# Jittor/JDet

Measured on AMD Instinct MI355X. Metric: img/s S2ANet-R50-FPN train step, 1024x1024 synthetic tiles, higher is better.
Workload: dtype f32; 1 GPU; s2anet_train; model=S2ANet-R50-FPN (configs/s2anet/s2anet_r50_fpn_1x_dota.py), global_batch=2, tile=1024x1024, gts_per_image=64, optimizer=SGD mom 0.9 wd 1e-4 clip 35 + StepLR warm-up (the config's lr), parallelism=dp1 (DDP, RCCL all-reduce)

## Files before the change

### jdet_amd/_lib.py

```python
import ctypes
import os
import subprocess

import torch

_HERE = os.path.dirname(os.path.abspath(__file__))
CSRC = os.path.join(_HERE, "csrc")
LIB_PATH = os.path.join(CSRC, "libjdet_hip.so")

_i, _f, _p, _sz, _l = ctypes.c_int, ctypes.c_float, ctypes.c_void_p, ctypes.c_size_t, ctypes.c_long



class BnParams(ctypes.Structure):
    _fields_ = [("weight", _p), ("bias", _p), ("mean", _p), ("var", _p), ("eps", _f)]


class ConvEpilogue(ctypes.Structure):
    _fields_ = [("mode", _i), ("affine", _i), ("relu", _i), ("bn", BnParams), ("residual", _p), ("grad_out", _p),
                ("act", _p), ("sums", _p)]


class BnSumsJob(ctypes.Structure):
    _fields_ = [("partial", _p), ("rows", _l), ("C", _i), ("gamma", _p), ("grad_gamma", _p), ("grad_beta", _p)]
# ... 98 lines not shown
    "jdet_rip_forward": (_i, [_p, _l, _i, _i, _p, _p]),
    "jdet_rip_backward": (_i, [_p, _p, _p, _l, _i, _i, _p, _p]),
    "jdet_delta2bbox_rotated": (_i, [_p, _p, _i, _i, _p, _p, _f, _p, _p]),
    "jdet_bbox2delta_rotated": (_i, [_p, _p, _i, _p, _p, _p, _p]),
    "jdet_midpoint_offset_decode": (_i, [_p, _p, _l, _p, _p, _f, _p, _p]),
    "jdet_midpoint_offset_encode": (_i, [_p, _p, _l, _p, _p, _p, _p]),
    "jdet_oriented_delta_decode": (_i, [_p, _p, _l, _i, _p, _p, _f, _p, _p]),
    "jdet_oriented_delta_encode": (_i, [_p, _p, _l, _p, _p, _p, _p]),
    "jdet_gliding_targets": (_i, [_p, _p, _l, _p, _p, _p, _p, _p, _p]),
    "jdet_gliding_decode": (_i, [_p, _p, _p, _p, _l, _i, _p, _p, _f, _f, _f, _f, _p, _p, _p]),
    "jdet_gv_delta_encode": (_i, [_p, _p, _l, _p, _p, _p, _p]),
    "jdet_gv_delta_decode": (_i, [_p, _p, _l, _i, _p, _p, _f, _f, _f, _p, _p]),
    "jdet_anchor_targets_rotated": (_i, [_p, _p, _p, _p, _i, _i, _p, _p, _f, _p, _p, _p, _p, _p, _p]),
    "jdet_anchor_targets_rotated_boxes": (_i, [_p, _p, _p, _i, _i, _f, _p, _p, _p, _p, _p, _p]),
    "jdet_obb2hbb2obb": (_i, [_p, _i, _i, _p, _p]),
    "jdet_assign_max_iou_workspace": (_sz, [_i]),
    "jdet_assign_max_iou": (_i, [_p, _i, _i, _f, _f, _f, _f, _i, _i, _p, _i, _p, _p, _p, _p, _sz, _p]),
}

ATSS_SIGNATURES = {
    "jdet_atss_assign_workspace": (_sz, [_i, _i, _i, _i]),
    "jdet_atss_assign": (_i, [_p, _i, _i, _p, _i, _p, _i, _p, _p, _i, _i, _p, _p, _p, _p, _sz, _p]),
}

ROWS_SIGNATURES = {
    "jdet_rows_nonzero_workspace": (_sz, [_i, _i, _i]),
    "jdet_rows_nonzero": (_i, [_p, _i, _i, _i, _i, _p, _p, _p, _p, _p, _sz, _p]),
    "jdet_conv3x3_rows_supported": (_i, [_i, _i]),
    "jdet_conv3x3_wgrad_rows_workers": (_i, [_i, _i]),
    "jdet_conv3x3_wgrad_rows": (_i, [_p, _p, _p, _p, _i, _i, _i, _i, _i, _p, _p]),
    "jdet_conv3x3_dgrad_rows": (_i, [_p, _p, _p, _p, _i, _i, _i, _i, _i, _i, _p, _p]),
}

FCOS_SIGNATURES = {
    "jdet_fcos_targets": (_i, [_p, _p, _i, _p, _p, _p, _i, _i, _i, _i, _i, _f, _p, _p, _p, _p, _p]),
    "jdet_poly_iou_loss": (_i, [_p, _p, _p, _l, _i, _f, _p, _p, _p]),
}

_lib = None

REFERENCE_SORT = 0


def build(force=False, verbose=False):
    cmd = ["make", "-C", CSRC, "-j8"] + (["-B"] if force else [])
    r = subprocess.run(cmd, capture_output=True, text=True)
    if r.returncode != 0:
        raise RuntimeError("building libjdet_hip.so failed:\n" + r.stdout[-4000:] + r.stderr[-4000:])
    if verbose:
        print(r.stdout[-2000:])
    return LIB_PATH


def lib():
    global _lib
    if _lib is None:
        if not os.path.exists(LIB_PATH):
            raise RuntimeError(
                "jdet_amd: %s not found.  Build it with `python -c 'import __graft_entry__ as g; g.build()'` "
                "or `make -C jdet_amd/csrc` (needs hipcc).  There is no CPU fallback." % LIB_PATH)
        l = ctypes.CDLL(LIB_PATH)
        for name, (res, args) in list(SIGNATURES.items()) + list(ATSS_SIGNATURES.items()) + list(ROWS_SIGNATURES.items()) + \
                list(FCOS_SIGNATURES.items()):
            fn = getattr(l, name)
            fn.restype = res
            fn.argtypes = args
        _lib = l
    return _lib


class JDetHipError(RuntimeError):
    pass


_ERR = {-1: "bad argument", -2: "unsupported shape", -3: "workspace too small"}


def check(status, what):
    if status != 0:
        msg = _ERR.get(status, "hipError_t %d" % status)
        raise JDetHipError("%s failed: %s" % (what, msg))


def stream_ptr(t=None):
    if t is not None and t.is_cuda and t.device.index != torch.cuda.current_device():
        torch.cuda.set_device(t.device)
    return torch.cuda.current_stream(t.device if t is not None else None).cuda_stream


def need_device(*tensors):
    for t in tensors:
        if t is None:
            continue
        if not t.is_cuda:
            raise JDetHipError(
                "jdet_amd ops run only on a HIP device (got a %s tensor); there is no CPU fallback "
# ... 53 lines not shown
```

### jdet_amd/csrc/conv_rows.hip

```cpp
#include "conv_mfma.h"
#include "jdet_hip_rows.h"

namespace {

constexpr int kBlk = 256;
constexpr int kFlagRows = 64;

typedef unsigned v4u __attribute__((ext_vector_type(4)));

__global__ __launch_bounds__(256) void rows_flag_kernel(const float* __restrict__ g, long P, int C4,
                                                        uint8_t* __restrict__ flags) {
  const int lane = threadIdx.x & 63, wave = threadIdx.x >> 6;
  const long base = (long)blockIdx.x * kFlagRows + wave * (kFlagRows / 4);
  const v4u* g4 = reinterpret_cast<const v4u*>(g);
  for (int r = 0; r < kFlagRows / 4; r += 4) {
    unsigned acc[4] = {0u, 0u, 0u, 0u};
#pragma unroll
    for (int u = 0; u < 4; u++) {
      const long row = base + r + u;
      if (row < P)
        for (int c = lane; c < C4; c += 64) {
          const v4u v = g4[row * C4 + c];
          acc[u] |= (v[0] | v[1] | v[2] | v[3]) & 0x7fffffffu;
        }
    }
#pragma unroll
    for (int u = 0; u < 4; u++) {
      const long row = base + r + u;
      const bool any = __ballot(acc[u] != 0u) != 0ull;
      if (lane == 0 && row < P) flags[row] = any ? 1 : 0;
    }
  }
}

// ... 226 lines not shown
#pragma unroll
    for (int i = 0; i < TM; i++)
#pragma unroll
      for (int j = 0; j < TN; j++) {
        const unsigned ci = (unsigned)(n0 + wn * 32 * TN + j * 32 + (lane & 31));
        const unsigned co = (unsigned)(m0 + wm * 32 * TM + i * 32 + 4 * (lane >> 5));
        const unsigned base = ((co * 9u + (unsigned)tap) * (unsigned)a.Cin + ci) * 4u;
#pragma unroll
        for (int e = 0; e < 16; e++)
          __builtin_amdgcn_raw_ptr_buffer_atomic_fadd_f32(acc[i][j][e], rgw, (int)base, (int)(cd_row(e) * row_bytes), 0);
      }
    return;
  }
#pragma unroll
  for (int i = 0; i < TM; i++)
#pragma unroll
    for (int j = 0; j < TN; j++) {
      const int ci = n0 + wn * 32 * TN + j * 32 + (lane & 31);
#pragma unroll
      for (int e = 0; e < 16; e++) {
        const int co = m0 + wm * 32 * TM + i * 32 + cd_row(e) + 4 * (lane >> 5);
        if (co < a.Cout && ci < a.Cin) unsafeAtomicAdd(a.gw + ((size_t)co * 9 + tap) * a.Cin + ci, acc[i][j][e]);
      }
    }
}

struct DgradRowsArgs {
  const float* g;
  const float* wd;
  const int* rows;
  const int* count;
  float* gx;
  int N, H, W, Cin, Cout;
};

template <int BK, int KG>
__global__ __launch_bounds__(256 * KG) __attribute__((amdgpu_waves_per_eu(4)))
void conv3x3_dgrad_rows_kernel(DgradRowsArgs a) {
  constexpr int BT = 64;
  constexpr int DEPTH = KG >= 1 ? 1 : 2;
  using TL = MfmaTile<BT, BK, KG>;
  constexpr int T = TL::T, CH = TL::CH, RPP = TL::RPP, PASSES = TL::PASSES, TILE = TL::TILE, QN = TL::QN;
  static_assert(T == 1, "64 x 64 tile");
  __shared__ __attribute__((aligned(16))) char s_raw[4 * TILE];
  const int tid = threadIdx.x, lane = tid & 63, wave = tid >> 6;
  const int P = a.N * a.H * a.W;
  const int KC = a.Cout, NO = a.Cin;
  int cnt = a.count[0];
  cnt = cnt < 0 ? 0 : (cnt > P ? P : cnt);
  const int NT = (NO + BT - 1) / BT;
  const int mtile = (int)((unsigned)blockIdx.x / (unsigned)NT);
  const int m0 = mtile * BT;
  if (m0 >= cnt) return;
  const int n0 = (blockIdx.x - mtile * NT) * BT;
  const __amdgpu_buffer_rsrc_t rx =
      __builtin_amdgcn_make_buffer_rsrc((void*)a.g, 0, (unsigned)((long)P * KC * 4), 0x00020000);
  const __amdgpu_buffer_rsrc_t rw =
      __builtin_amdgcn_make_buffer_rsrc((void*)a.wd, 0, (unsigned)((long)NO * 9 * KC * 4), 0x00020000);
  const int lchunk = tid % CH, lrow = tid / CH;
  int img[PASSES], py[PASSES], px[PASSES];
  bool m_ok[PASSES];
  unsigned wv[PASSES];
  int st_off[PASSES];
  const unsigned hw = (unsigned)(a.H * a.W);
#pragma unroll
  for (int p = 0; p < PASSES; p++) {
    const int row = p * RPP + lrow;
    const int li = m0 + row;
    const unsigned pos = li < cnt ? (unsigned)a.rows[li] : 0xFFFFFFFFu;
// ... 50 lines not shown
    fb_off[qq] = TILE + swz_bytes<BK>(wn * (BT / 2) + frow, chunk);
  }
  v16f acc[T][T];
#pragma unroll
  for (int e = 0; e < 16; e++) acc[0][0][e] = 0.f;

  int tap = 0, c = 0;
  set_tap(0);
  auto advance = [&]() {
    c += BK;
    if (c == KC) {
      c = 0;
      tap++;
      set_tap(tap);
    }
  };
  auto mfma_step = [&](int buf) { ::mfma_step<BT, BK, KG>(s_raw, buf, fa_off, fb_off, acc); };
#include "conv_mfma_loop.inc"
  if (KG == 2) {
    float* red = reinterpret_cast<float*>(s_raw);
    if (kg == 1) {
#pragma unroll
      for (int e = 0; e < 16; e++) red[red_index<T>(wave, lane, 0, 0, e)] = acc[0][0][e];
    }
    __syncthreads();
    if (kg == 1) return;
  }

  const __amdgpu_buffer_rsrc_t ry =
      __builtin_amdgcn_make_buffer_rsrc((void*)a.gx, 0, (unsigned)((long)P * NO * 4), 0x00020000);
  const int lrow0 = m0 + wm * (BT / 2) + 4 * (lane >> 5);
  const int n = n0 + wn * (BT / 2) + (lane & 31);
  unsigned dst[16];
#pragma unroll
  for (int e = 0; e < 16; e++) {
    const int li = lrow0 + cd_row(e);
    const unsigned pos = li < cnt ? (unsigned)a.rows[li] : 0xFFFFFFFFu;
    dst[e] = (pos < (unsigned)P && n < NO) ? (pos * (unsigned)NO + (unsigned)n) * 4u : kOob;
  }
#pragma unroll
  for (int e = 0; e < 16; e++) {
    float v = acc[0][0][e];
    if (KG == 2) v += reinterpret_cast<const float*>(s_raw)[red_index<T>(wave, lane, 0, 0, e)];
    __builtin_amdgcn_raw_buffer_store_b32(__builtin_bit_cast(unsigned, v), ry, dst[e], 0u, 0);
  }
}

inline size_t align16(size_t v) { return (v + 15) & ~(size_t)15; }

inline int wgrad_rows_workers(int Cin, int Cout) {
  const int tm = Cout > 64 ? 2 : 1;
  const long tiles = (long)((Cout + 64 * tm - 1) / (64 * tm)) * ((Cin + 63) / 64) * 9;
  long kw = 1152 / tiles;
  return (int)(kw < 8 ? 8 : (kw > 64 ? 64 : kw));
}

}

JDET_API size_t jdet_rows_nonzero_workspace(int N, int H, int W) {
  if (N <= 0 || H <= 0 || W <= 0) return 0;
  const long P = (long)N * H * W;
  const long nb = (P + kBlk - 1) / kBlk;
  return align16((size_t)P) + sizeof(int32_t) * 2 * (size_t)nb;
}

JDET_API int jdet_rows_nonzero(const float* g_nhwc, int N, int H, int W, int C, uint8_t* flags, int32_t* rows,
                               int32_t* rows_dilated, int32_t* counts, void* workspace, size_t workspace_bytes,
                               jdet_stream_t stream) {
  if (N <= 0 || H <= 0 || W <= 0 || C <= 0) return JDET_E_BADARG;
  if (C % 4 != 0) return JDET_E_UNSUPPORTED;
  const long P = (long)N * H * W;
  if (P * C >= (1L << 30)) return JDET_E_UNSUPPORTED;
  if (!g_nhwc || !flags || !rows || !rows_dilated || !counts) return JDET_E_BADARG;
  if (((uintptr_t)g_nhwc & 15) || (((uintptr_t)rows | (uintptr_t)rows_dilated | (uintptr_t)counts) & 3))
    return JDET_E_BADARG;
  if (!workspace || workspace_bytes < jdet_rows_nonzero_workspace(N, H, W)) return JDET_E_WORKSPACE;
// ... 23 lines not shown
                                     const int32_t* count, int N, int H, int W, int Cin, int Cout, float* gw_krsc,
                                     jdet_stream_t stream) {
  if (N <= 0 || H <= 0 || W <= 0 || Cin <= 0 || Cout <= 0) return JDET_E_BADARG;
  if (!jdet_conv3x3_rows_supported(Cin, Cout)) return JDET_E_UNSUPPORTED;
  const long P = (long)N * H * W;
  if ((P + BKW) * (Cin > Cout ? Cin : Cout) >= (1L << 30)) return JDET_E_UNSUPPORTED;
  if (!x_nhwc || !gy_nhwc || !rows || !count || !gw_krsc) return JDET_E_BADARG;
  if ((((uintptr_t)x_nhwc) | ((uintptr_t)gy_nhwc)) & 15 || (((uintptr_t)rows | (uintptr_t)count) & 3)) return JDET_E_BADARG;
  const int tm = Cout > 64 ? 2 : 1;
  const int kw = wgrad_rows_workers(Cin, Cout);
  const unsigned grid = (unsigned)(((Cout + 64 * tm - 1) / (64 * tm)) * ((Cin + 63) / 64) * 9 * kw);
  WgradRowsArgs a{x_nhwc, gy_nhwc, rows, count, gw_krsc, N, H, W, Cin, Cout, kw};
  hipStream_t st = (hipStream_t)stream;
  if (tm == 2) hipLaunchKernelGGL((conv3x3_wgrad_rows_kernel<2>), dim3(grid), dim3(256), 0, st, a);
  else hipLaunchKernelGGL((conv3x3_wgrad_rows_kernel<1>), dim3(grid), dim3(256), 0, st, a);
  return jdet_launch_status();
}

JDET_API int jdet_conv3x3_dgrad_rows(const float* gy_nhwc, const float* wd_crsk, const int32_t* rows,
                                     const int32_t* count, int N, int H, int W, int Cin, int Cout, int zero_first,
                                     float* gx_nhwc, jdet_stream_t stream) {
  if (N <= 0 || H <= 0 || W <= 0 || Cin <= 0 || Cout <= 0) return JDET_E_BADARG;
  if (!jdet_conv3x3_rows_supported(Cin, Cout)) return JDET_E_UNSUPPORTED;
  const long P = (long)N * H * W;
  if (P * (Cin > Cout ? Cin : Cout) >= (1L << 30)) return JDET_E_UNSUPPORTED;
  if (!gy_nhwc || !wd_crsk || !rows || !count || !gx_nhwc) return JDET_E_BADARG;
  if ((((uintptr_t)gy_nhwc) | ((uintptr_t)wd_crsk)) & 15 || (((uintptr_t)rows | (uintptr_t)count | (uintptr_t)gx_nhwc) & 3))
    return JDET_E_BADARG;
  hipStream_t st = (hipStream_t)stream;
  if (zero_first) {
    const int e = jdet_zero_async(gx_nhwc, sizeof(float) * (size_t)P * Cin, st);
    if (e) return e;
  }
  DgradRowsArgs a{gy_nhwc, wd_crsk, rows, count, gx_nhwc, N, H, W, Cin, Cout};
  const unsigned grid = (unsigned)(((P + 63) / 64) * ((Cin + 63) / 64));
  if (Cout % 32 == 0) hipLaunchKernelGGL((conv3x3_dgrad_rows_kernel<32, 2>), dim3(grid), dim3(512), 0, st, a);
  else hipLaunchKernelGGL((conv3x3_dgrad_rows_kernel<16, 1>), dim3(grid), dim3(256), 0, st, a);
  return jdet_launch_status();
}
```

### jdet_amd/models/roi_heads/s2anet_head.py

```python
import os

import torch
from torch import nn
try:
    from torch.nn.utils.stateless import _reparametrize_module
except ImportError:
    _reparametrize_module = None

from jdet_amd.models.boxes.anchor_generator import AnchorGeneratorRotatedS2ANet
from jdet_amd.models.boxes.anchor_target import anchor_target, images_to_levels
from jdet_amd.models.boxes.box_ops import delta2bbox_rotated
from jdet_amd.models.utils.level_pack import LevelPack

HEAD_STREAMS = os.environ.get("JDET_HEAD_STREAMS", "0") == "1"
FUSED_PACK_MASK = os.environ.get("JDET_PACK_FUSED_MASK", "1") == "1"
_SIDE = {}


def _side_stream(device):
    s = _SIDE.get(device)
    if s is None:
        s = _SIDE[device] = torch.cuda.Stream(device)
    return s
from jdet_amd.models.utils.modules import ConvModule
# ... 109 lines not shown
        normal_init(self.fam_reg, std=0.01)
        normal_init(self.fam_cls, std=0.01, bias=bias_cls)
        self.align_conv.init_weights()
        normal_init(self.or_conv, std=0.01)
        for m in self.odm_reg_convs:
            normal_init(m.conv, std=0.01)
        for m in self.odm_cls_convs:
            normal_init(m.conv, std=0.01)
        normal_init(self.odm_cls, std=0.01, bias=bias_cls)
        normal_init(self.odm_reg, std=0.01)

    def _towers(self, x, convs, mask=None, rows=None):
        for conv in convs:
            y = conv.masked(x, rows) if rows is not None and hasattr(conv, "masked") else None
            if y is not None:
                x = y
                continue
            x = conv(x)
            if mask is not None:
                x = x * mask
        return x

    def _fam(self, x, mask=None, rows=None):
        fam_bbox_pred = conv_module(self.fam_reg, self._towers(x, self.fam_reg_convs, mask, rows))
        fam_cls_score = conv_module(self.fam_cls, self._towers(x, self.fam_cls_convs, mask, rows)) if self.training else None
        return fam_cls_score, fam_bbox_pred

    def _refine(self, x, fam_bbox_pred, stride):
        num_level = self.anchor_strides.index(stride)
        init_anchors = self._init_anchors(num_level, tuple(fam_bbox_pred.shape[-2:]), x.device)
        refine_anchor = bbox_decode(fam_bbox_pred.detach(), init_anchors, self.target_means, self.target_stds)
        return refine_anchor, self.align_conv(x, refine_anchor, stride)

    def _odm(self, align_feat, mask=None, rows=None):
        or_feat = self.or_conv(align_feat)
        if mask is not None:
            or_feat = or_feat * mask
        odm_cls_feat = self.or_pool(or_feat) if self.with_orconv else or_feat
        odm_cls_score = conv_module(self.odm_cls, self._towers(odm_cls_feat, self.odm_cls_convs, mask, rows))
        odm_bbox_pred = conv_module(self.odm_reg, self._towers(or_feat, self.odm_reg_convs, mask, rows))
        return odm_cls_score, odm_bbox_pred

    def forward_single(self, x, stride):
        fam_cls_score, fam_bbox_pred = self._fam(x)
        refine_anchor, align_feat = self._refine(x, fam_bbox_pred, stride)
        odm_cls_score, odm_bbox_pred = self._odm(align_feat)
        return fam_cls_score, fam_bbox_pred, refine_anchor, odm_cls_score, odm_bbox_pred

    def forward_packed(self, xs, strides):
        pack = LevelPack.cached([tuple(x.shape[-2:]) for x in xs], xs[0].device)
        mask = pack.mask.to(xs[0].dtype)
        rows = pack.row_mask(xs[0].shape[0]) if FUSED_PACK_MASK and xs[0].dtype == torch.float32 else None
        fam_cls_p, fam_box_p = self._fam(pack.pack(xs), mask, rows)
        fam_box = pack.unpack(fam_box_p)
        fam_cls = pack.unpack(fam_cls_p) if fam_cls_p is not None else [None] * len(xs)
        refined = [self._refine(x, b, stride) for x, b, stride in zip(xs, fam_box, strides)]
        odm_cls_p, odm_box_p = self._odm(pack.pack([r[1] for r in refined]), mask, rows)
        odm_cls, odm_box = pack.unpack(odm_cls_p), pack.unpack(odm_box_p)
        return [(fam_cls[i], fam_box[i], refined[i][0], odm_cls[i], odm_box[i]) for i in range(len(xs))]

    def get_refine_anchors(self, featmap_sizes, refine_anchors, img_metas, is_train=True, device=None):
        num_levels = len(featmap_sizes)
        refine_anchors_list = []
        for img_id in range(len(img_metas)):
            refine_anchors_list.append([refine_anchors[i][img_id].reshape(-1, 5) for i in range(num_levels)])
        valid_flag_list = self._valid_flags(featmap_sizes, img_metas, device) if is_train else []
        return refine_anchors_list, valid_flag_list

    def loss(self, fam_cls_scores, fam_bbox_preds, refine_anchors, odm_cls_scores, odm_bbox_preds, gt_bboxes,
             gt_labels, img_metas, gt_bboxes_ignore=None):
        cfg = self.train_cfg.copy()
        featmap_sizes = [tuple(featmap.shape[-2:]) for featmap in odm_cls_scores]
        assert len(featmap_sizes) == len(self.anchor_generators)
        device = odm_cls_scores[0].device
        anchor_list, valid_flag_list = self.get_init_anchors(featmap_sizes, img_metas, device)
        num_level_anchors = [anchors.size(0) for anchors in anchor_list[0]]
        need_anchors = cfg.fam_cfg.get("reg_decoded_bbox", False) or cfg.odm_cfg.get("reg_decoded_bbox", False)
        all_anchor_list = [None] * len(num_level_anchors)
        if need_anchors:
            concat_anchor_list = [torch.cat(anchor_list[i]) for i in range(len(anchor_list))]
            all_anchor_list = images_to_levels(concat_anchor_list, num_level_anchors)

        label_channels = self.cls_out_channels if self.use_sigmoid_cls else 1
        cls_reg_targets = anchor_target(anchor_list, valid_flag_list, gt_bboxes, img_metas, self.target_means,
                                        self.target_stds, cfg.fam_cfg, gt_bboxes_ignore_list=gt_bboxes_ignore,
                                        gt_labels_list=gt_labels, label_channels=label_channels,
                                        sampling=self.sampling)
        if cls_reg_targets is None:
            return None
        labels_list, label_weights_list, bbox_targets_list, bbox_weights_list, num_total_pos, num_total_neg = \
            cls_reg_targets
        num_total_samples = num_total_pos + num_total_neg if self.sampling else num_total_pos
        losses_fam_cls, losses_fam_bbox = multi_apply(
            self.loss_fam_single, fam_cls_scores, fam_bbox_preds, all_anchor_list, labels_list, label_weights_list,
            bbox_targets_list, bbox_weights_list, num_total_samples=num_total_samples, cfg=cfg.fam_cfg)

        refine_anchors_list, valid_flag_list = self.get_refine_anchors(featmap_sizes, refine_anchors, img_metas,
                                                                       device=device)
        num_level_anchors = [anchors.size(0) for anchors in refine_anchors_list[0]]
        all_anchor_list = [None] * len(num_level_anchors)
        if need_anchors:
            concat_anchor_list = [torch.cat(refine_anchors_list[i]) for i in range(len(refine_anchors_list))]
            all_anchor_list = images_to_levels(concat_anchor_list, num_level_anchors)
        cls_reg_targets = anchor_target(refine_anchors_list, valid_flag_list, gt_bboxes, img_metas, self.target_means,
                                        self.target_stds, cfg.odm_cfg, gt_bboxes_ignore_list=gt_bboxes_ignore,
                                        gt_labels_list=gt_labels, label_channels=label_channels,
                                        sampling=self.sampling)
        if cls_reg_targets is None:
            return None
        (labels_list, label_weights_list, bbox_targets_list, bbox_weights_list, num_total_pos, num_total_neg) = \
            cls_reg_targets
        num_total_samples = num_total_pos + num_total_neg if self.sampling else num_total_pos
        losses_odm_cls, losses_odm_bbox = multi_apply(
            self.loss_odm_single, odm_cls_scores, odm_bbox_preds, all_anchor_list, labels_list, label_weights_list,
            bbox_targets_list, bbox_weights_list, num_total_samples=num_total_samples, cfg=cfg.odm_cfg)
        return dict(loss_fam_cls=losses_fam_cls, loss_fam_bbox=losses_fam_bbox, loss_odm_cls=losses_odm_cls,
                    loss_odm_bbox=losses_odm_bbox)

    def loss_fam_single(self, fam_cls_score, fam_bbox_pred, anchors, labels, label_weights, bbox_targets,
                        bbox_weights, num_total_samples, cfg):
        return self._loss_single(self.loss_fam_cls, self.loss_fam_bbox, fam_cls_score, fam_bbox_pred, anchors, labels,
                                 label_weights, bbox_targets, bbox_weights, num_total_samples, cfg)

    def loss_odm_single(self, odm_cls_score, odm_bbox_pred, anchors, labels, label_weights, bbox_targets,
                        bbox_weights, num_total_samples, cfg):
        return self._loss_single(self.loss_odm_cls, self.loss_odm_bbox, odm_cls_score, odm_bbox_pred, anchors, labels,
                                 label_weights, bbox_targets, bbox_weights, num_total_samples, cfg)

    def get_bboxes(self, fam_cls_scores, fam_bbox_preds, refine_anchors, odm_cls_scores, odm_bbox_preds, img_metas,
                   rescale=True):
        assert len(odm_cls_scores) == len(odm_bbox_preds)
        cfg = self.test_cfg.copy()
        featmap_sizes = [tuple(featmap.shape[-2:]) for featmap in odm_cls_scores]
        num_levels = len(odm_cls_scores)
        refine_anchors = self.get_refine_anchors(featmap_sizes, refine_anchors, img_metas, is_train=False)
        result_list = []
        for img_id in range(len(img_metas)):
            cls_score_list = [odm_cls_scores[i][img_id].detach() for i in range(num_levels)]
            bbox_pred_list = [odm_bbox_preds[i][img_id].detach() for i in range(num_levels)]
            img_shape = img_metas[img_id]["img_shape"]
# ... 3 lines not shown
        return result_list

    def _level_outputs(self, feats):
        small = [i for i, f in enumerate(feats)
                 if f.is_cuda and f.shape[-2] * f.shape[-1] <= self.pack_max_positions]
        outs = [None] * len(feats)
        side = None
        if len(small) >= 2:
            if (HEAD_STREAMS and _reparametrize_module is not None and len(small) < len(feats)
                    and torch.is_grad_enabled() and not torch.cuda.is_current_stream_capturing()):
                side = _side_stream(feats[0].device)
                main = torch.cuda.current_stream(feats[0].device)
                side.wait_stream(main)
            if side is not None:
                alias = {n: p.view_as(p) for n, p in self.named_parameters() if p.requires_grad}
                with torch.cuda.stream(side), _reparametrize_module(self, alias):
                    packed = self.forward_packed([feats[i] for i in small], [self.anchor_strides[i] for i in small])
            else:
                packed = self.forward_packed([feats[i] for i in small], [self.anchor_strides[i] for i in small])
            for i, o in zip(small, packed):
                outs[i] = o
        for i, f in enumerate(feats):
            if outs[i] is None:
                outs[i] = self.forward_single(f, self.anchor_strides[i])
        if side is not None:
            main.wait_stream(side)
            for i in small:
                feats[i].record_stream(side)
                for t in outs[i]:
                    if torch.is_tensor(t):
                        t.record_stream(main)
        return tuple(map(list, zip(*outs)))

    def forward(self, feats, targets):
        outs = self._level_outputs(feats)
        if self.training:
            return self.loss(*outs, *self.parse_targets(targets))
        return self.get_bboxes(*outs, self.parse_targets(targets, is_train=False))

    execute = forward


def bbox_decode(bbox_preds, anchors, means=[0, 0, 0, 0, 0], stds=[1, 1, 1, 1, 1]):
    num_imgs, _, H, W = bbox_preds.shape
    deltas = bbox_preds.permute(0, 2, 3, 1).reshape(num_imgs * H * W, 5)
    rois = anchors.unsqueeze(0).expand(num_imgs, H * W, 5).reshape(num_imgs * H * W, 5)
    bboxes = delta2bbox_rotated(rois, deltas, means, stds, wh_ratio_clip=1e-6)
    return bboxes.reshape(num_imgs, H, W, 5)


class AlignConv(nn.Module):
    def __init__(self, in_channels, out_channels, kernel_size=3, deformable_groups=1):
        super().__init__()
        self.kernel_size = kernel_size
        self.deform_conv = DeformConv(in_channels, out_channels, kernel_size=kernel_size,
                                      padding=(kernel_size - 1) // 2, deformable_groups=deformable_groups)
        self.relu = nn.ReLU()

    def init_weights(self):
        normal_init(self.deform_conv, std=0.01)

    @torch.no_grad()
    def get_offset(self, anchors, featmap_size, stride):
        dtype, device = anchors.dtype, anchors.device
        feat_h, feat_w = featmap_size
        if anchors.is_cuda and dtype == torch.float32:
            from jdet_amd import _lib as L
# ... 37 lines not shown
```

### jdet_amd/ops/conv_igemm.py

```python
import os
import weakref

import torch

from jdet_amd import _lib as L


def supported(cin, cout):
    return bool(L.lib().jdet_conv3x3_igemm_supported(int(cin), int(cout)))


def weight_krsc(weight):
    return L.f32c(weight.permute(0, 2, 3, 1))


def conv3x3_nhwc(x_nhwc, w_krsc, bias=None, relu=False, rowmask=None, offset=None, tile=0):
    L.need_device(x_nhwc, w_krsc, bias, rowmask, offset)
    N, H, W, Cin = x_nhwc.shape
    Cout = w_krsc.shape[0]
    if w_krsc.shape[1:] != (3, 3, Cin):
        raise ValueError("weight %r does not match input channels %d" % (tuple(w_krsc.shape), Cin))
    if offset is not None and tuple(offset.shape) != (N, 18, H, W):
        raise ValueError("offset must be (N, 18, H, W), got %r" % (tuple(offset.shape),))
    x_nhwc, w_krsc = L.f32c(x_nhwc), L.f32c(w_krsc)
# ... 238 lines not shown
        out = torch.empty((N, H, W, Cin), dtype=torch.float32, device=gy_nhwc.device)
    L.check(L.lib().jdet_conv3x3_dgrad_rows(L.ptr(gy_nhwc), L.ptr(wd_crsk), L.ptr(rows), count_ptr, N, H, W, Cin, Cout,
                                            int(zero), L.ptr(out), L.stream_ptr(gy_nhwc)), "jdet_conv3x3_dgrad_rows")
    return out


def _rows_dgrad_weight(weight):
    if torch.cuda.is_current_stream_capturing() or not weight.is_cuda:
        return weight.detach().flip(2, 3).permute(1, 2, 3, 0).contiguous()
    wd = dgrad_weight(weight)
    st = _DGRAD_BANKS.get(weight.device)
    if st is None or st["bank"] is None or id(weight) not in st["items"]:
        return dgrad_weight_fresh(weight)
    tid = torch._C._current_graph_task_id()
    if tid < 0 or st.get("pass") != tid:
        st["bank"].refresh()
        st["pass"] = tid
    return wd


def dgrad_weight_fresh(weight):
    return weight.detach().flip(2, 3).permute(1, 2, 3, 0).contiguous()


def _rows_backward(g, x, weight, need_x, need_w):
    gn, xn = L.f32c(g.permute(0, 2, 3, 1)), L.f32c(x.permute(0, 2, 3, 1))
    _, rows, drows, counts = rows_nonzero(gn)
    gx = gw = None
    if need_w:
        gw = shared_wgrad(weight, xn, gn, rows=(rows, counts.data_ptr()))
    if need_x:
        gx = conv3x3_dgrad_rows_nhwc(gn, _rows_dgrad_weight(weight), drows, counts.data_ptr() + 4).permute(0, 3, 1, 2)
    return gx, gw


CONV1X1_GEMM = os.environ.get("JDET_CONV1X1_GEMM", "1") == "1"


def _is_1x1(x, weight, stride, padding, groups):
    return (CONV1X1_GEMM and tuple(weight.shape[2:]) == (1, 1) and tuple(stride) == (1, 1) and tuple(padding) == (0, 0)
            and groups == 1 and x.is_cuda and x.dtype == torch.float32 and weight.shape[0] >= 64
            and x.is_contiguous(memory_format=torch.channels_last))


class _ConvBiasAct(torch.autograd.Function):

    @staticmethod
    def forward(ctx, x, weight, bias, relu, stride, padding, dilation, groups, igemm, rowmask=None, row_sparse=False):
        k1 = _is_1x1(x, weight, stride, padding, groups)
        if igemm:
            y = conv3x3_nhwc(L.f32c(x.permute(0, 2, 3, 1)), weight_krsc(weight), bias, relu,
                             rowmask).permute(0, 3, 1, 2)
        elif k1 and weight.shape[1] >= 256 and x.shape[0] * x.shape[2] * x.shape[3] <= 32768:
            N, Ci, H, W = x.shape
            Co = weight.shape[0]
            xm = x.permute(0, 2, 3, 1).reshape(-1, Ci)
            ym = torch.addmm(bias, xm, weight.view(Co, Ci).t()) if bias is not None else xm @ weight.view(Co, Ci).t()
            if relu:
                ym = torch.relu_(ym)
            y = ym.view(N, H, W, Co).permute(0, 3, 1, 2)
        else:
            y = torch.ops.aten.convolution(x, weight, bias, stride, padding, dilation, False, [0, 0], groups)
            if relu:
                y = torch.relu_(y)
        ctx.k1 = k1
        ctx.row_sparse = bool(row_sparse) and bool(igemm)
# ... 95 lines not shown
```

Before: 84.64 img/s.

## Compute ODM regression tower only at rows needed by positive targets

Training now computes the ODM anchor targets before the regression tower. It derives per-position flags from the bbox weights and dilates them into row lists, then runs the odm_reg 3x3 convs only on those rows, using a forward variant of the row-sparse dgrad kernel with bias, ReLU and rowmask fused in. The aim is to skip most of the forward FLOPs of the reg tower, since only positions near positive anchors affect the loss. This reorders target assignment ahead of the head. It assumes outputs outside the dilated rows never reach the loss, and it adds the flag-to-rows kernel launches.

```diff
diff --git a/include/jdet_hip_rows_fwd.h b/include/jdet_hip_rows_fwd.h
--- /dev/null
+++ b/include/jdet_hip_rows_fwd.h
@@ -0,0 +1,24 @@
+#ifndef JDET_HIP_ROWS_FWD_H_
+#define JDET_HIP_ROWS_FWD_H_
+
+#include "jdet_hip.h"
+
+#ifdef __cplusplus
+extern "C" {
+#endif
+
+size_t jdet_rows_from_flags_workspace(int N, int H, int W);
+int jdet_rows_from_flags(const uint8_t* flags, int N, int H, int W, int32_t* rows, int32_t* rows_dilated,
+                         int32_t* rows_dilated2, int32_t* counts, void* workspace, size_t workspace_bytes,
+                         jdet_stream_t stream);
+
+int jdet_conv3x3_rows_forward_supported(int Cin, int Cout);
+
+int jdet_conv3x3_rows_forward(const float* x_nhwc, const float* w_krsc, const float* bias, int relu,
+                              const float* rowmask, const int32_t* rows, const int32_t* count, int N, int H, int W,
+                              int Cin, int Cout, int zero_first, float* y_nhwc, jdet_stream_t stream);
+
+#ifdef __cplusplus
+}
+#endif
+#endif
diff --git a/jdet_amd/_lib.py b/jdet_amd/_lib.py
--- a/jdet_amd/_lib.py
+++ b/jdet_amd/_lib.py
@@ -154,6 +154,13 @@
     "jdet_conv3x3_dgrad_rows": (_i, [_p, _p, _p, _p, _i, _i, _i, _i, _i, _i, _p, _p]),
 }
 
+ROWS_FWD_SIGNATURES = {
+    "jdet_rows_from_flags_workspace": (_sz, [_i, _i, _i]),
+    "jdet_rows_from_flags": (_i, [_p, _i, _i, _i, _p, _p, _p, _p, _p, _sz, _p]),
+    "jdet_conv3x3_rows_forward_supported": (_i, [_i, _i]),
+    "jdet_conv3x3_rows_forward": (_i, [_p, _p, _p, _i, _p, _p, _p, _i, _i, _i, _i, _i, _i, _p, _p]),
+}
+
 FCOS_SIGNATURES = {
     "jdet_fcos_targets": (_i, [_p, _p, _i, _p, _p, _p, _i, _i, _i, _i, _i, _f, _p, _p, _p, _p, _p]),
     "jdet_poly_iou_loss": (_i, [_p, _p, _p, _l, _i, _f, _p, _p, _p]),
@@ -183,7 +190,7 @@
                 "or `make -C jdet_amd/csrc` (needs hipcc).  There is no CPU fallback." % LIB_PATH)
         l = ctypes.CDLL(LIB_PATH)
         for name, (res, args) in list(SIGNATURES.items()) + list(ATSS_SIGNATURES.items()) + list(ROWS_SIGNATURES.items()) + \
-                list(FCOS_SIGNATURES.items()):
+                list(ROWS_FWD_SIGNATURES.items()) + list(FCOS_SIGNATURES.items()):
             fn = getattr(l, name)
             fn.restype = res
             fn.argtypes = args
diff --git a/jdet_amd/csrc/conv_rows.hip b/jdet_amd/csrc/conv_rows.hip
--- a/jdet_amd/csrc/conv_rows.hip
+++ b/jdet_amd/csrc/conv_rows.hip
@@ -1,5 +1,6 @@
 #include "conv_mfma.h"
 #include "jdet_hip_rows.h"
+#include "jdet_hip_rows_fwd.h"
 
 namespace {
 
@@ -292,9 +293,12 @@
   const int* count;
   float* gx;
   int N, H, W, Cin, Cout;
+  const float* bias;
+  const float* rowmask;
+  int relu;
 };
 
-template <int BK, int KG>
+template <int BK, int KG, bool FWD>
 __global__ __launch_bounds__(256 * KG) __attribute__((amdgpu_waves_per_eu(4)))
 void conv3x3_dgrad_rows_kernel(DgradRowsArgs a) {
   constexpr int BT = 64;
@@ -411,16 +415,25 @@
   const int lrow0 = m0 + wm * (BT / 2) + 4 * (lane >> 5);
   const int n = n0 + wn * (BT / 2) + (lane & 31);
   unsigned dst[16];
+  float mk[16];
+  float b = 0.f;
+  if constexpr (FWD) b = (a.bias && n < NO) ? a.bias[n] : 0.f;
 #pragma unroll
   for (int e = 0; e < 16; e++) {
     const int li = lrow0 + cd_row(e);
     const unsigned pos = li < cnt ? (unsigned)a.rows[li] : 0xFFFFFFFFu;
     dst[e] = (pos < (unsigned)P && n < NO) ? (pos * (unsigned)NO + (unsigned)n) * 4u : kOob;
+    if constexpr (FWD) mk[e] = (a.rowmask && pos < (unsigned)P) ? a.rowmask[pos] : 1.f;
   }
 #pragma unroll
   for (int e = 0; e < 16; e++) {
     float v = acc[0][0][e];
     if (KG == 2) v += reinterpret_cast<const float*>(s_raw)[red_index<T>(wave, lane, 0, 0, e)];
+    if constexpr (FWD) {
+      v += b;
+      if (a.relu) v = fmaxf(v, 0.f);
+      if (a.rowmask) v *= mk[e];
+    }
     __builtin_amdgcn_raw_buffer_store_b32(__builtin_bit_cast(unsigned, v), ry, dst[e], 0u, 0);
   }
 }
@@ -510,9 +523,70 @@
     const int e = jdet_zero_async(gx_nhwc, sizeof(float) * (size_t)P * Cin, st);
     if (e) return e;
   }
-  DgradRowsArgs a{gy_nhwc, wd_crsk, rows, count, gx_nhwc, N, H, W, Cin, Cout};
+  DgradRowsArgs a{gy_nhwc, wd_crsk, rows, count, gx_nhwc, N, H, W, Cin, Cout, nullptr, nullptr, 0};
   const unsigned grid = (unsigned)(((P + 63) / 64) * ((Cin + 63) / 64));
-  if (Cout % 32 == 0) hipLaunchKernelGGL((conv3x3_dgrad_rows_kernel<32, 2>), dim3(grid), dim3(512), 0, st, a);
-  else hipLaunchKernelGGL((conv3x3_dgrad_rows_kernel<16, 1>), dim3(grid), dim3(256), 0, st, a);
+  if (Cout % 32 == 0) hipLaunchKernelGGL((conv3x3_dgrad_rows_kernel<32, 2, false>), dim3(grid), dim3(512), 0, st, a);
+  else hipLaunchKernelGGL((conv3x3_dgrad_rows_kernel<16, 1, false>), dim3(grid), dim3(256), 0, st, a);
   return jdet_launch_status();
 }
+
+
+JDET_API size_t jdet_rows_from_flags_workspace(int N, int H, int W) {
+  if (N <= 0 || H <= 0 || W <= 0) return 0;
+  const long P = (long)N * H * W;
+  const long nb = (P + kBlk - 1) / kBlk;
+  return 2 * align16((size_t)P) + sizeof(int32_t) * 4 * (size_t)nb;
+}
+
+JDET_API int jdet_rows_from_flags(const uint8_t* flags, int N, int H, int W, int32_t* rows, int32_t* rows_dilated,
+                                  int32_t* rows_dilated2, int32_t* counts, void* workspace, size_t workspace_bytes,
+                                  jdet_stream_t stream) {
+  if (N <= 0 || H <= 0 || W <= 0) return JDET_E_BADARG;
+  const long P = (long)N * H * W;
+  if (P >= (1L << 30)) return JDET_E_UNSUPPORTED;
+  if (!flags || !rows || !rows_dilated || !rows_dilated2 || !counts) return JDET_E_BADARG;
+  if (((uintptr_t)rows | (uintptr_t)rows_dilated | (uintptr_t)rows_dilated2 | (uintptr_t)counts) & 3) return JDET_E_BADARG;
+  if (!workspace || workspace_bytes < jdet_rows_from_flags_workspace(N, H, W)) return JDET_E_WORKSPACE;
+  if ((uintptr_t)workspace & 3) return JDET_E_BADARG;
+  hipStream_t st = (hipStream_t)stream;
+  const unsigned nb = (unsigned)((P + kBlk - 1) / kBlk);
+  uint8_t* d1 = (uint8_t*)workspace;
+  uint8_t* d2 = d1 + align16((size_t)P);
+  int* c0 = (int*)(d2 + align16((size_t)P));
+  int* c1 = c0 + nb;
+  int* c1b = c1 + nb;
+  int* c2 = c1b + nb;
+  hipLaunchKernelGGL(rows_dilate_kernel, dim3(nb), dim3(256), 0, st, flags, H, W, P, d1, c0, c1);
+  hipLaunchKernelGGL(rows_dilate_kernel, dim3(nb), dim3(256), 0, st, (const uint8_t*)d1, H, W, P, d2, c1b, c2);
+  hipLaunchKernelGGL(rows_list_kernel, dim3(nb), dim3(256), 0, st, flags, (const uint8_t*)d1, P, (const int*)c0,
+                     (const int*)c1, rows, rows_dilated, counts);
+  hipLaunchKernelGGL(rows_list_kernel, dim3(nb), dim3(256), 0, st, (const uint8_t*)d1, (const uint8_t*)d2, P,
+                     (const int*)c1b, (const int*)c2, rows_dilated, rows_dilated2, counts + 1);
+  return jdet_launch_status();
+}
+
+JDET_API int jdet_conv3x3_rows_forward_supported(int Cin, int Cout) {
+  return Cin > 0 && Cout > 0 && Cin % 16 == 0 && Cout % 16 == 0;
+}
+
+JDET_API int jdet_conv3x3_rows_forward(const float* x_nhwc, const float* w_krsc, const float* bias, int relu,
+                                       const float* rowmask, const int32_t* rows, const int32_t* count, int N, int H,
+                                       int W, int Cin, int Cout, int zero_first, float* y_nhwc, jdet_stream_t stream) {
+  if (N <= 0 || H <= 0 || W <= 0 || Cin <= 0 || Cout <= 0) return JDET_E_BADARG;
+  if (!jdet_conv3x3_rows_forward_supported(Cin, Cout)) return JDET_E_UNSUPPORTED;
+  const long P = (long)N * H * W;
+  if (P * (Cin > Cout ? Cin : Cout) >= (1L << 30)) return JDET_E_UNSUPPORTED;
+  if (!x_nhwc || !w_krsc || !rows || !count || !y_nhwc) return JDET_E_BADARG;
+  if ((((uintptr_t)x_nhwc) | ((uintptr_t)w_krsc)) & 15) return JDET_E_BADARG;
+  if (((uintptr_t)rows | (uintptr_t)count | (uintptr_t)y_nhwc | (uintptr_t)bias | (uintptr_t)rowmask) & 3) return JDET_E_BADARG;
+  hipStream_t st = (hipStream_t)stream;
+  if (zero_first) {
+    const int e = jdet_zero_async(y_nhwc, sizeof(float) * (size_t)P * Cout, st);
+    if (e) return e;
+  }
+  DgradRowsArgs a{x_nhwc, w_krsc, rows, count, y_nhwc, N, H, W, Cout, Cin, bias, rowmask, relu ? 1 : 0};
+  const unsigned grid = (unsigned)(((P + 63) / 64) * ((Cout + 63) / 64));
+  if (Cin % 32 == 0) hipLaunchKernelGGL((conv3x3_dgrad_rows_kernel<32, 2, true>), dim3(grid), dim3(512), 0, st, a);
+  else hipLaunchKernelGGL((conv3x3_dgrad_rows_kernel<16, 1, true>), dim3(grid), dim3(256), 0, st, a);
+  return jdet_launch_status();
+}
diff --git a/jdet_amd/models/roi_heads/s2anet_head.py b/jdet_amd/models/roi_heads/s2anet_head.py
--- a/jdet_amd/models/roi_heads/s2anet_head.py
+++ b/jdet_amd/models/roi_heads/s2anet_head.py
@@ -165,12 +165,16 @@
         refine_anchor = bbox_decode(fam_bbox_pred.detach(), init_anchors, self.target_means, self.target_stds)
         return refine_anchor, self.align_conv(x, refine_anchor, stride)
 
-    def _odm(self, align_feat, mask=None, rows=None):
+    def _odm_front(self, align_feat, mask=None, rows=None):
         or_feat = self.or_conv(align_feat)
         if mask is not None:
             or_feat = or_feat * mask
         odm_cls_feat = self.or_pool(or_feat) if self.with_orconv else or_feat
         odm_cls_score = conv_module(self.odm_cls, self._towers(odm_cls_feat, self.odm_cls_convs, mask, rows))
+        return or_feat, odm_cls_score
+
+    def _odm(self, align_feat, mask=None, rows=None):
+        or_feat, odm_cls_score = self._odm_front(align_feat, mask, rows)
         odm_bbox_pred = conv_module(self.odm_reg, self._towers(or_feat, self.odm_reg_convs, mask, rows))
         return odm_cls_score, odm_bbox_pred
 
@@ -200,8 +204,16 @@
         valid_flag_list = self._valid_flags(featmap_sizes, img_metas, device) if is_train else []
         return refine_anchors_list, valid_flag_list
 
+    def _odm_targets(self, featmap_sizes, refine_anchors, gt_bboxes, gt_labels, img_metas, gt_bboxes_ignore, device):
+        refine_anchors_list, valid_flag_list = self.get_refine_anchors(featmap_sizes, refine_anchors, img_metas,
+                                                                       device=device)
+        label_channels = self.cls_out_channels if self.use_sigmoid_cls else 1
+        return anchor_target(refine_anchors_list, valid_flag_list, gt_bboxes, img_metas, self.target_means,
+                             self.target_stds, self.train_cfg.odm_cfg, gt_bboxes_ignore_list=gt_bboxes_ignore,
+                             gt_labels_list=gt_labels, label_channels=label_channels, sampling=self.sampling)
+
     def loss(self, fam_cls_scores, fam_bbox_preds, refine_anchors, odm_cls_scores, odm_bbox_preds, gt_bboxes,
-             gt_labels, img_metas, gt_bboxes_ignore=None):
+             gt_labels, img_metas, gt_bboxes_ignore=None, odm_targets=None):
         cfg = self.train_cfg.copy()
         featmap_sizes = [tuple(featmap.shape[-2:]) for featmap in odm_cls_scores]
         assert len(featmap_sizes) == len(self.anchor_generators)
@@ -235,10 +247,12 @@
         if need_anchors:
             concat_anchor_list = [torch.cat(refine_anchors_list[i]) for i in range(len(refine_anchors_list))]
             all_anchor_list = images_to_levels(concat_anchor_list, num_level_anchors)
-        cls_reg_targets = anchor_target(refine_anchors_list, valid_flag_list, gt_bboxes, img_metas, self.target_means,
-                                        self.target_stds, cfg.odm_cfg, gt_bboxes_ignore_list=gt_bboxes_ignore,
-                                        gt_labels_list=gt_labels, label_channels=label_channels,
-                                        sampling=self.sampling)
+        cls_reg_targets = odm_targets
+        if cls_reg_targets is None:
+            cls_reg_targets = anchor_target(refine_anchors_list, valid_flag_list, gt_bboxes, img_metas,
+                                            self.target_means, self.target_stds, cfg.odm_cfg,
+                                            gt_bboxes_ignore_list=gt_bboxes_ignore, gt_labels_list=gt_labels,
+                                            label_channels=label_channels, sampling=self.sampling)
         if cls_reg_targets is None:
             return None
         (labels_list, label_weights_list, bbox_targets_list, bbox_weights_list, num_total_pos, num_total_neg) = \
@@ -308,7 +322,80 @@
                         t.record_stream(main)
         return tuple(map(list, zip(*outs)))
 
+    def _rows_forward_route(self, feats):
+        from jdet_amd.ops import conv_igemm as CI
+        if not (self.training and torch.is_grad_enabled() and not HEAD_STREAMS and len(feats) > 0):
+            return False
+        for m in self.odm_reg_convs:
+            if (not isinstance(m, ConvModule) or m.with_norm or not m.with_activation or type(m.activate) is not nn.ReLU
+                    or m.order.index("conv") > m.order.index("act") or not m.row_sparse_grad):
+                return False
+        if type(self.odm_reg) is not nn.Conv2d or self.odm_reg.kernel_size != (3, 3) or self.odm_reg.padding != (1, 1):
+            return False
+        convs = [m.conv for m in self.odm_reg_convs]
+        if not all(f.dim() == 4 and CI.rows_tower_applicable(convs, f) for f in feats):
+            return False
+        small = [f for f in feats if f.shape[-2] * f.shape[-1] <= self.pack_max_positions]
+        if len(small) >= 2:
+            pack = LevelPack.cached([tuple(f.shape[-2:]) for f in small], small[0].device)
+            return CI.rows_tower_applicable(convs, small[0], small[0].shape[0] * pack.height * pack.width)
+        return True
+
+    def _forward_train_rows(self, feats, targets):
+        from jdet_amd.ops import conv_igemm as CI
+        gt_bboxes, gt_labels, img_metas, gt_bboxes_ignore = self.parse_targets(targets)
+        n = len(feats)
+        fam_cls, fam_box, refine, odm_cls, odm_box = ([None] * n for _ in range(5))
+        small = [i for i, f in enumerate(feats)
+                 if f.is_cuda and f.shape[-2] * f.shape[-1] <= self.pack_max_positions]
+        groups = []
+        if len(small) >= 2:
+            xs = [feats[i] for i in small]
+            pack = LevelPack.cached([tuple(x.shape[-2:]) for x in xs], xs[0].device)
+            mask = pack.mask.to(xs[0].dtype)
+            rows = pack.row_mask(xs[0].shape[0]) if FUSED_PACK_MASK and xs[0].dtype == torch.float32 else None
+            fam_cls_p, fam_box_p = self._fam(pack.pack(xs), mask, rows)
+            boxes, scores = pack.unpack(fam_box_p), pack.unpack(fam_cls_p)
+            refined = [self._refine(x, b, self.anchor_strides[i]) for x, b, i in zip(xs, boxes, small)]
+            or_feat, odm_cls_p = self._odm_front(pack.pack([r[1] for r in refined]), mask, rows)
+            for k, (i, c) in enumerate(zip(small, pack.unpack(odm_cls_p))):
+                fam_cls[i], fam_box[i], refine[i], odm_cls[i] = scores[k], boxes[k], refined[k][0], c
+            groups.append((small, pack, or_feat))
+        else:
+            small = []
+        for i, f in enumerate(feats):
+            if i in small:
+                continue
+            fam_cls[i], fam_box[i] = self._fam(f)
+            refine[i], align_feat = self._refine(f, fam_box[i], self.anchor_strides[i])
+            or_feat, odm_cls[i] = self._odm_front(align_feat)
+            groups.append(([i], None, or_feat))
+
+        featmap_sizes = [tuple(f.shape[-2:]) for f in feats]
+        odm_targets = self._odm_targets(featmap_sizes, refine, gt_bboxes, gt_labels, img_metas, gt_bboxes_ignore,
+                                        feats[0].device)
+        if odm_targets is None:
+            return None
+        num_imgs = feats[0].shape[0]
+        with torch.no_grad():
+            flags = [bw.reshape(num_imgs, h * w, -1).ne(0).any(-1) for bw, (h, w) in zip(odm_targets[3], featmap_sizes)]
+        convs = [m.conv for m in self.odm_reg_convs]
+        for levels, pack, or_feat in groups:
+            if pack is None:
+                odm_box[levels[0]] = conv_module(self.odm_reg, CI.rows_tower(convs, or_feat, flags[levels[0]]))
+                continue
+            canvas = torch.zeros((num_imgs, pack.height, pack.width), dtype=torch.bool, device=or_feat.device)
+            for i, (h, w), (r0, c0) in zip(levels, pack.sizes, pack.places):
+                canvas[:, r0:r0 + h, c0:c0 + w] = flags[i].view(num_imgs, h, w)
+            tower = CI.rows_tower(convs, or_feat, canvas, pack.row_mask(num_imgs))
+            for i, b in zip(levels, pack.unpack(conv_module(self.odm_reg, tower))):
+                odm_box[i] = b
+        return self.loss(fam_cls, fam_box, refine, odm_cls, odm_box, gt_bboxes, gt_labels, img_metas,
+                         gt_bboxes_ignore, odm_targets=odm_targets)
+
     def forward(self, feats, targets):
+        if self._rows_forward_route(feats):
+            return self._forward_train_rows(feats, targets)
         outs = self._level_outputs(feats)
         if self.training:
             return self.loss(*outs, *self.parse_targets(targets))
diff --git a/jdet_amd/ops/conv_igemm.py b/jdet_amd/ops/conv_igemm.py
--- a/jdet_amd/ops/conv_igemm.py
+++ b/jdet_amd/ops/conv_igemm.py
@@ -294,6 +294,89 @@
     if need_x:
         gx = conv3x3_dgrad_rows_nhwc(gn, _rows_dgrad_weight(weight), drows, counts.data_ptr() + 4).permute(0, 3, 1, 2)
     return gx, gw
+
+
+ROWS_FWD = os.environ.get("JDET_CONV_ROWS_FWD", "1") == "1"
+
+
+def rows_forward_supported(cin, cout):
+    return bool(L.lib().jdet_conv3x3_rows_forward_supported(int(cin), int(cout)))
+
+
+def rows_from_flags(flags, N, H, W):
+    L.need_device(flags)
+    P = N * H * W
+    if flags.numel() != P or flags.element_size() != 1 or not flags.is_contiguous():
+        raise ValueError("flags must be %d contiguous bytes, got %r %s" % (P, tuple(flags.shape), flags.dtype))
+    wsb = L.lib().jdet_rows_from_flags_workspace(N, H, W)
+    buf = torch.empty((12 * P + 16 + wsb,), dtype=torch.uint8, device=flags.device)
+    rows = [buf[4 * i * P:4 * (i + 1) * P].view(torch.int32) for i in range(3)]
+    counts = buf[12 * P:12 * P + 12].view(torch.int32)
+    ws = buf[12 * P + 16:]
+    L.check(L.lib().jdet_rows_from_flags(L.ptr(flags), N, H, W, L.ptr(rows[0]), L.ptr(rows[1]), L.ptr(rows[2]),
+                                         L.ptr(counts), L.ptr(ws), wsb, L.stream_ptr(flags)), "jdet_rows_from_flags")
+    return rows[0], rows[1], rows[2], counts
+
+
+def conv3x3_rows_forward_nhwc(x_nhwc, w_krsc, bias, relu, rowmask, rows, count_ptr, out=None):
+    L.need_device(x_nhwc, w_krsc, bias, rowmask, rows, out)
+    N, H, W, Cin = x_nhwc.shape
+    Cout = w_krsc.shape[0]
+    if tuple(w_krsc.shape[1:]) != (3, 3, Cin):
+        raise ValueError("weight %r does not match input channels %d" % (tuple(w_krsc.shape), Cin))
+    x_nhwc, w_krsc = L.f32c(x_nhwc), L.f32c(w_krsc)
+    zero = out is None
+    if zero:
+        out = torch.empty((N, H, W, Cout), dtype=torch.float32, device=x_nhwc.device)
+    L.check(L.lib().jdet_conv3x3_rows_forward(
+        L.ptr(x_nhwc), L.ptr(w_krsc), L.ptr(L.f32c(bias)) if bias is not None else None, int(bool(relu)),
+        L.ptr(L.f32c(rowmask)) if rowmask is not None else None, L.ptr(rows), count_ptr, N, H, W, Cin, Cout, int(zero),
+        L.ptr(out), L.stream_ptr(x_nhwc)), "jdet_conv3x3_rows_forward")
+    return out
+
+
+class _ConvBiasActRows(torch.autograd.Function):
+
+    @staticmethod
+    def forward(ctx, x, weight, bias, relu, rowmask, rows, count_ptr):
+        y = conv3x3_rows_forward_nhwc(L.f32c(x.permute(0, 2, 3, 1)), weight_krsc(weight), bias, relu, rowmask, rows,
+                                      count_ptr).permute(0, 3, 1, 2)
+        ctx.k1 = False
+        ctx.row_sparse = True
+        ctx.cfg = (bool(relu), [1, 1], [1, 1], [1, 1], 1, True, bias is not None)
+        ctx.save_for_backward(x, weight, y if relu else None)
+        return y
+
+    @staticmethod
+    def backward(ctx, g):
+        return _ConvBiasAct.backward(ctx, g)[:7]
+
+
+def rows_tower_applicable(convs, x, positions=None):
+    if not (ROWS and ROWS_FWD and TRAIN and BIAS_ACT_BWD and 1 <= len(convs) <= 2):
+        return False
+    if not (x.is_cuda and x.dtype == torch.float32 and x.dim() == 4) or torch.is_autocast_enabled():
+        return False
+    for conv in convs:
+        if not (type(conv).__name__ == "Conv2d" and conv.padding_mode == "zeros" and not isinstance(conv.padding, str)
+                and _is_igemm_conv(conv) and conv.weight.dtype == torch.float32 and conv.bias is not None
+                and conv.bias.requires_grad and _bias_bwd_supported(conv.out_channels)
+                and rows_forward_supported(conv.in_channels, conv.out_channels)
+                and rows_supported(conv.in_channels, conv.out_channels)):
+            return False
+    P = x.shape[0] * x.shape[2] * x.shape[3] if positions is None else positions
+    return (P + 16) * max([c.in_channels for c in convs] + [c.out_channels for c in convs]) < 2 ** 30
+
+
+def rows_tower(convs, x, flags, rowmask=None):
+    N, _, H, W = x.shape
+    lists = rows_from_flags(flags, N, H, W)
+    counts = lists[3]
+    n = len(convs)
+    for i, conv in enumerate(convs):
+        k = n - i
+        x = _ConvBiasActRows.apply(x, conv.weight, conv.bias, True, rowmask, lists[k], counts.data_ptr() + 4 * k)
+    return x
 
 
 CONV1X1_GEMM = os.environ.get("JDET_CONV1X1_GEMM", "1") == "1"
```

New measurement: 86.63 img/s (median of 6 runs). 2.4% higher.
